# AlexandreRouma/SDRPlusPlus

Hardware: NVIDIA H100
Metric: complex IQ MSamples/s through FFT + 8-VFO WFM chain (higher is better)
Workload: dtype f32

## Files before the change

sdrplusplus_b200/csrc/api.cpp:

```cpp
#include "../../include/b200dsp.h"
#include "engine.h"
#include <chrono>
#include <map>
#include <cmath>
#include <cstdio>
#include <cstring>
#include <cstdlib>
#include <algorithm>

using namespace b200;

static int g_device = -1;

static int ensure_device() {
    int n = 0;
    cudaError_t e = cudaGetDeviceCount(&n);
    if (e != cudaSuccess || n <= 0) {
        set_error("no usable CUDA device (%s): libb200dsp has no CPU fallback", e == cudaSuccess ? "0 devices" : cudaGetErrorString(e));
        cudaGetLastError();
        return B200_ENODEV;
    }
    if (g_device < 0) { g_device = 0; }
    B200_CK(cudaSetDevice(g_device));
    return 0;
// ... 55 lines not shown
extern "C" int b200_resamp_plan_get(double inSR, double outSR, b200_resamp_plan* out) {
    if (!out) { set_error("null plan"); return B200_EINVAL; }
    ResampPlan pl = make_resamp_plan(inSR, outSR);
    memset(out, 0, sizeof(*out));
    out->mode = pl.mode;
    out->predec_ratio = pl.predec_ratio;
    out->interp = pl.interp;
    out->decim = pl.decim;
    out->ntaps = (int)pl.rtaps.size();
    out->taps_per_phase = pl.taps_per_phase;
    if (pl.use_decim) {
        const DecimPlan* dp = find_decim_plan(pl.predec_ratio);
        if (!dp) { set_error("no decimation plan for ratio %d", pl.predec_ratio); return B200_ENOPLAN; }
        out->nstages = (int)dp->stages.size();
        for (int i = 0; i < out->nstages && i < 8; i++) {
            out->stage_decim[i] = dp->stages[i].decim;
            out->stage_taps[i] = (int)dp->stages[i].taps.size();
        }
    }
    return 0;
}

static int bytes_per_sample(int fmt) { return fmt == B200_FMT_CF32 ? 8 : (fmt == B200_FMT_CS16 ? 4 : 2); }
static int ilog2(int n) { int l = 0; while ((1 << l) < n) { l++; } return l; }

struct FftCore {
    FftPlanDev plan;
    DevBuf tw, twf, win, work;
    int size = 0, nz = 0, window = 0;
    int create(int size_, int nz_, int window_, int max_batch = 1) {
        if (size_ < 8 || size_ > (1 << 22) || (size_ & (size_ - 1))) { set_error("FFT size %d must be a power of two in [8, 4194304]", size_); return B200_EINVAL; }
        if (nz_ < 1 || nz_ > size_) { set_error("bad nz %d", nz_); return B200_EINVAL; }
        size = size_; nz = nz_; window = window_;
        memset(&plan, 0, sizeof(plan));
        plan.N = size; plan.logN = ilog2(size);
        if (size <= 8192) { plan.N1 = size; plan.logN1 = plan.logN; plan.N2 = 1; plan.logN2 = 0; }
        else {
            plan.logN1 = (plan.logN + 1) / 2; plan.N1 = 1 << plan.logN1;
            plan.logN2 = plan.logN - plan.logN1; plan.N2 = 1 << plan.logN2;
        }
        plan.TW = std::max(plan.N1, plan.N2); plan.logTW = ilog2(plan.TW);
        std::vector<float2> t((size_t)plan.TW);
        for (int k = 0; k < plan.TW; k++) {
            double a = -2.0 * 3.14159265358979323846 * (double)k / (double)plan.TW;
            t[k] = make_float2((float)std::cos(a), (float)std::sin(a));
        }
        int rc;
        if ((rc = tw.alloc(t.size() * sizeof(float2)))) { return rc; }
        B200_CK(cudaMemcpy(tw.p, t.data(), t.size() * sizeof(float2), cudaMemcpyHostToDevice));
        std::vector<float> w = fft_window(window, nz);
        if ((rc = win.alloc((size_t)nz * sizeof(float)))) { return rc; }
        B200_CK(cudaMemcpy(win.p, w.data(), (size_t)nz * sizeof(float), cudaMemcpyHostToDevice));
        if ((rc = work.alloc((size_t)size * sizeof(float2) * (size_t)(max_batch > 0 ? max_batch : 1)))) { return rc; }
        plan.tw = tw.as<float2>(); plan.window = win.as<float>(); plan.nz = nz;
        plan.tw_fine = nullptr;
        if (plan.N2 > 1) {
            const int nf = size / plan.TW;
            std::vector<float2> f((size_t)nf);
            for (int j = 0; j < nf; j++) {
                double a = -2.0 * 3.14159265358979323846 * (double)j / (double)size;
                f[j] = make_float2((float)std::cos(a), (float)std::sin(a));
            }
            if ((rc = twf.alloc(f.size() * sizeof(float2)))) { return rc; }
            B200_CK(cudaMemcpy(twf.p, f.data(), f.size() * sizeof(float2), cudaMemcpyHostToDevice));
            plan.tw_fine = twf.as<float2>();
        }
        B200_CK(cudaDeviceSynchronize());
        return 0;
    }
};

struct VfoSlot {
    bool used = false;
    b200_vfo_cfg cfg;
    Chain chain;
    bool pend_offset = false, pend_bw = false;
    double new_offset = 0, new_bw = 0;
};

#define FE_SLOTS 4

struct b200_fe {
    double fs = 0;
    int max_chunk = 0;
    Scheduler sch;
    cudaStream_t own_stream = nullptr, copy_stream = nullptr, fft_stream = nullptr, tail_stream = nullptr, join_stream = nullptr;
    cudaEvent_t ev_tail_done[FE_SLOTS] = {};
    cudaEvent_t ev_fft_go = nullptr, ev_fft_done = nullptr, ev_lines_free = nullptr;
    bool overlap = true;
    bool lines_busy = false;
    float* lines_override = nullptr;
    bool fft_async = true;
    bool fft_join_pending = false;
    std::vector<std::unique_ptr<VfoSlot>> vfos;
    std::mutex mtx;
    DevBuf in_dev[FE_SLOTS];
    bool fft_on = false;
    FftCore fft;
    double fft_rate = 0;
    int skip = 0;
    DevBuf frame, lines;
    int max_lines = 0;
    unsigned long long pos = 0, fstart = 0;
    cudaEvent_t ev_h2d[FE_SLOTS] = {}, ev_compute[FE_SLOTS] = {}, ev_out[FE_SLOTS] = {};
    bool slot_used[FE_SLOTS] = {};
    int max_inflight = 2;
    unsigned long long nsub = 0, nwait = 0;
    int fft_serial = 0;
    int host_direct = -1;
    long long host_ns[4] = { 0, 0, 0, 0 };
    float scale16 = 1.0f / 32768.0f, scale8 = 1.0f / 128.0f;
    int decim = 1;
    double fs_eff = 0;
    bool dc_block = false, invert_iq = false;
    Chain pre;
    Scheduler sch_pre;
    DevBuf pp[FE_SLOTS];
    DevBuf dc_state, dc_segA, dc_segB;
    int max_eff = 0;
};

static float fe_ingest_scale(const b200_fe* fe, int fmt) {
    if (fmt == B200_FMT_CS16) { return fe->scale16; }
    if (fmt == B200_FMT_CS8) { return fe->scale8; }
    return 0.0f;
}

static int fe_alloc_fft(b200_fe* fe) {
    int rc;
    if ((rc = fe->frame.alloc((size_t)fe->fft.nz * sizeof(float2)))) { return rc; }
    long long interval = (long long)fe->fft.nz + fe->skip;
    fe->max_lines = (int)(fe->max_eff / interval) + 2;
    return fe->lines.alloc((size_t)fe->max_lines * fe->fft.size * sizeof(float));
}

extern "C" b200_fe* b200_fe_create(double samplerate, int max_chunk) {
    if (ensure_device()) { return nullptr; }
    if (samplerate <= 0 || max_chunk < 1) { set_error("bad samplerate/max_chunk"); return nullptr; }
    b200_fe* fe = new b200_fe;
    fe->fs = samplerate;
    fe->fs_eff = samplerate;
    fe->max_chunk = max_chunk;
    fe->max_eff = max_chunk;
    int lo = 0, hi = 0;
    cudaDeviceGetStreamPriorityRange(&lo, &hi);
    int pt = 2, pm = 1, pf = 0;
    if (const char* e = getenv("B200_STREAM_PRIO")) { sscanf(e, "%d,%d,%d", &pt, &pm, &pf); }
    if (const char* e = getenv("B200_FFT_SERIAL")) { fe->fft_serial = atoi(e); }
    if (const char* e = getenv("B200_FFT_CTA")) { kernels_set_fft_cta(atoi(e)); }
    auto prio = [&](int level) { int p = lo - level; return p < hi ? hi : p; };
    bool ok = cudaStreamCreateWithPriority(&fe->own_stream, cudaStreamNonBlocking, prio(pm)) == cudaSuccess &&
              cudaStreamCreateWithFlags(&fe->copy_stream, cudaStreamNonBlocking) == cudaSuccess &&
              cudaStreamCreateWithPriority(&fe->fft_stream, cudaStreamNonBlocking, prio(pf)) == cudaSuccess &&
              cudaStreamCreateWithPriority(&fe->tail_stream, cudaStreamNonBlocking, prio(pt)) == cudaSuccess &&
              cudaStreamCreateWithFlags(&fe->join_stream, cudaStreamNonBlocking) == cudaSuccess &&
              cudaEventCreateWithFlags(&fe->ev_lines_free, cudaEventDisableTiming) == cudaSuccess &&
              cudaEventCreateWithFlags(&fe->ev_fft_go, cudaEventDisableTiming) == cudaSuccess &&
              cudaEventCreateWithFlags(&fe->ev_fft_done, cudaEventDisableTiming) == cudaSuccess;
    for (int i = 0; i < FE_SLOTS && ok; i++) {
        ok = cudaEventCreateWithFlags(&fe->ev_h2d[i], cudaEventDisableTiming) == cudaSuccess &&
             cudaEventCreateWithFlags(&fe->ev_compute[i], cudaEventDisableTiming) == cudaSuccess &&
             cudaEventCreateWithFlags(&fe->ev_tail_done[i], cudaEventDisableTiming) == cudaSuccess &&
             cudaEventCreateWithFlags(&fe->ev_out[i], cudaEventDisableTiming) == cudaSuccess;
    }
    if (!ok || fe->sch.init_raw()) {
        if (ok) {} else { cuda_fail(cudaGetLastError(), "stream/event creation"); }
        b200_fe_destroy(fe);
        return nullptr;
    }
    fe->sch.stream = fe->own_stream;
    fe->sch.fuse.on = true;
    kernels_set_xd_tma_stages(2);
    kernels_set_xd_tma_diag(0);
    {
        int dev = 0, sms = 0;
        if (cudaGetDevice(&dev) == cudaSuccess && cudaDeviceGetAttribute(&sms, cudaDevAttrMultiProcessorCount, dev) == cudaSuccess && sms > 0) {
            fe->sch.sm_count = sms;
        }
    }
    if (fe->sch.enable_overlap(fe->tail_stream)) { b200_fe_destroy(fe); return nullptr; }
    return fe;
}

extern "C" void b200_fe_destroy(b200_fe* fe) {
    if (!fe) { return; }
    cudaDeviceSynchronize();
    for (int i = 0; i < FE_SLOTS; i++) {
        if (fe->ev_h2d[i]) { cudaEventDestroy(fe->ev_h2d[i]); }
        if (fe->ev_compute[i]) { cudaEventDestroy(fe->ev_compute[i]); }
        if (fe->ev_tail_done[i]) { cudaEventDestroy(fe->ev_tail_done[i]); }
        if (fe->ev_out[i]) { cudaEventDestroy(fe->ev_out[i]); }
    }
    if (fe->ev_lines_free) { cudaEventDestroy(fe->ev_lines_free); }
    if (fe->tail_stream) { cudaStreamDestroy(fe->tail_stream); }
    if (fe->join_stream) { cudaStreamDestroy(fe->join_stream); }
    for (int i = 0; i < 2; i++) {
        if (fe->sch.ev_stage1[i]) { cudaEventDestroy(fe->sch.ev_stage1[i]); }
        if (fe->sch.ev_tail[i]) { cudaEventDestroy(fe->sch.ev_tail[i]); }
    }
    if (fe->ev_fft_go) { cudaEventDestroy(fe->ev_fft_go); }
    if (fe->ev_fft_done) { cudaEventDestroy(fe->ev_fft_done); }
    if (fe->own_stream) { cudaStreamDestroy(fe->own_stream); }
// ... 162 lines not shown
    if (!v) { return B200_EINVAL; }
    return v->chain.max_out(count);
}
extern "C" int b200_fe_fft_max_lines(b200_fe* fe, int count) {
    if (!fe || !fe->fft_on) { return 0; }
    return (int)(count / ((long long)fe->fft.nz + fe->skip)) + 2;
}
extern "C" long long b200_fe_launch_count(b200_fe* fe) { return fe ? fe->sch.launches : 0; }
extern int g_xd_tma_launches;
extern "C" long long b200_fe_stat(b200_fe* fe, const char* key) {
    if (!fe || !key) { return -1; }
    if (!strcmp(key, "launches")) { return fe->sch.launches; }
    if (!strcmp(key, "s1_tma_launches")) { return g_xd_tma_launches; }
    if (!strcmp(key, "chunks")) { return (long long)fe->nsub; }
    if (!strcmp(key, "host_ns_plan")) { return fe->host_ns[0]; }
    if (!strcmp(key, "host_ns_fft")) { return fe->host_ns[1]; }
    if (!strcmp(key, "host_ns_run")) { return fe->host_ns[2]; }
    if (!strcmp(key, "host_ns_join")) { return fe->host_ns[3]; }
    if (!strcmp(key, "graph_hits")) { return fe->sch.graph_hits; }
    if (!strcmp(key, "graph_misses")) { return fe->sch.graph_misses; }
    if (!strcmp(key, "graphs")) { return (long long)fe->sch.graphs.size(); }
    if (!strcmp(key, "host_ns_stage1")) { return fe->sch.host_ns[0]; }
    if (!strcmp(key, "host_ns_tail")) { return fe->sch.host_ns[1]; }
    return -1;
}
extern "C" int b200_fe_set_option(b200_fe* fe, const char* key, int value) {
    if (!fe || !key) { set_error("null argument"); return B200_EINVAL; }
    if (!strcmp(key, "s1")) { fe->sch.s1_variant = value; return 0; }
    if (!strcmp(key, "overlap")) {
        if (b200_fe_vfo_count(fe) > 0) { set_error("'overlap' must be chosen before VFOs are added"); return B200_ESTATE; }
        if (cudaDeviceSynchronize() != cudaSuccess) { return cuda_fail(cudaGetLastError(), "sync"); }
        fe->sch.tail_stream = value ? fe->tail_stream : nullptr;
        return 0;
    }
    if (!strcmp(key, "pair")) { fe->sch.pair_conjugates = value != 0; return 0; }
    if (!strcmp(key, "fft_async")) { fe->fft_async = value != 0; return 0; }
    if (!strcmp(key, "s1_mt")) { kernels_set_xd_tile(value); return 0; }
    if (!strcmp(key, "s1_cps")) { kernels_set_xd_cps(value); return 0; }
    if (!strcmp(key, "s1_stages")) { kernels_set_xd_tma_stages(value); return 0; }
    if (!strcmp(key, "s1_diag")) { kernels_set_xd_tma_diag(value); return 0; }
    if (!strcmp(key, "s1_ctas")) { kernels_set_xd_tma_ctas(value); return 0; }
    if (!strcmp(key, "tails") || !strncmp(key, "ft_", 3)) {
        if (b200_fe_vfo_count(fe) > 0) { set_error("'%s' must be chosen before VFOs are added", key); return B200_ESTATE; }
        if (!strcmp(key, "tails")) { kernels_set_tail_variant(value >= 1 ? 1 : 0); fe->sch.fuse.on = value >= 2; return 0; }
        if (!strcmp(key, "ft_ob")) { fe->sch.fuse.ob_force = value; return 0; }
        if (!strcmp(key, "ft_obmax")) { fe->sch.fuse.ob_max = value; return 0; }
        if (!strcmp(key, "ft_smem_kb")) { fe->sch.fuse.smem_limit = value * 1024; return 0; }
        if (!strcmp(key, "ft_threads")) { fe->sch.fuse.threads = value; return 0; }
        if (!strcmp(key, "ft_direct")) { fe->sch.fuse.direct = value != 0; return 0; }
        if (!strcmp(key, "ft_prereg")) { fe->sch.fuse.pre_reg = value; return 0; }
        if (!strcmp(key, "ft_regall")) { fe->sch.fuse.reg_all = value != 0; return 0; }
    }
    if (!strcmp(key, "fft")) { kernels_set_fft_variant(value); return 0; }
    if (!strcmp(key, "fft_cta")) { kernels_set_fft_cta(value); return 0; }
    if (!strcmp(key, "host_direct")) { fe->host_direct = value; return 0; }
    if (!strcmp(key, "inflight")) {
        if (value < 1 || value > FE_SLOTS) { set_error("inflight: 1 ... %d", FE_SLOTS); return B200_EINVAL; }
        fe->max_inflight = value;
        return 0;
    }
    if (!strcmp(key, "fft_serial")) { fe->fft_serial = value; return 0; }
    if (!strcmp(key, "graph")) { fe->sch.graph_tails = value; if (value == 0) { fe->sch.drop_graphs(); } return 0; }
    if (!strcmp(key, "graph_max_count")) { fe->sch.graph_max_count = value; return 0; }
    if (!strcmp(key, "pdl")) { kernels_set_pdl(value); fe->sch.drop_graphs(); return 0; }
    if (!strcmp(key, "tail_split")) { fe->sch.tail_split = value; fe->sch.drop_graphs(); return 0; }
    if (!strcmp(key, "time_s1")) { fe->sch.time_s1 = value != 0; for (auto& t : fe->sch.timers) { t.used = 0; } return 0; }
    set_error("unknown option %s", key);
    return B200_EINVAL;
}

extern "C" int b200_fe_s1_stats(b200_fe* fe, double* ms_total, int* launches) {
    if (!fe || !ms_total || !launches) { set_error("null argument"); return B200_EINVAL; }
    return fe->sch.s1_stats(ms_total, launches);
}
extern "C" int b200_fe_group_stats(b200_fe* fe, int group, double* ms_total, int* launches) {
    if (!fe || !ms_total || !launches) { set_error("null argument"); return B200_EINVAL; }
    return fe->sch.group_stats(group, ms_total, launches);
}

extern "C" int b200_fe_reset(b200_fe* fe) {
    if (!fe) { set_error("null fe"); return B200_EINVAL; }
    std::lock_guard<std::mutex> lck(fe->mtx);
    B200_CK(cudaDeviceSynchronize());
    for (auto& v : fe->vfos) {
        if (v->used) { v->chain.reset_state(); }
    }
    int rc = fe->sch.reset_raw();
    if (!fe->pre.st.empty()) { fe->pre.reset_state(); }
    if (fe->dc_state.p) { B200_CK(cudaMemset(fe->dc_state.p, 0, 16)); B200_CK(cudaDeviceSynchronize()); }
    fe->pos = 0;
    fe->fstart = 0;
    return rc;
}

static std::mutex g_host_mtx;
static std::map<uintptr_t, size_t> g_host_allocs;
static bool host_buffer_is_ours(const void* p, size_t bytes) {
    std::lock_guard<std::mutex> lk(g_host_mtx);
    auto it = g_host_allocs.upper_bound((uintptr_t)p);
    if (it == g_host_allocs.begin()) { return false; }
    --it;
    return (uintptr_t)p + bytes <= it->first + it->second;
}

static inline long long host_clock_ns() {
    return (long long)std::chrono::duration_cast<std::chrono::nanoseconds>(std::chrono::steady_clock::now().time_since_epoch()).count();
}
// ... 1071 lines not shown
```

sdrplusplus_b200/csrc/fft_reg.cuh:

```cuda
#pragma once

__device__ constexpr float FR_COS[16] = { 1.000000000e+00f, 9.807852804e-01f, 9.238795325e-01f, 8.314696123e-01f, 7.071067812e-01f, 5.555702330e-01f,
                                          3.826834324e-01f, 1.950903220e-01f, 0.0f, -1.950903220e-01f, -3.826834324e-01f, -5.555702330e-01f,
                                          -7.071067812e-01f, -8.314696123e-01f, -9.238795325e-01f, -9.807852804e-01f };
__device__ constexpr float FR_SIN[16] = { 0.000000000e+00f, 1.950903220e-01f, 3.826834324e-01f, 5.555702330e-01f, 7.071067812e-01f, 8.314696123e-01f,
                                          9.238795325e-01f, 9.807852804e-01f, 1.0f, 9.807852804e-01f, 9.238795325e-01f, 8.314696123e-01f,
                                          7.071067812e-01f, 5.555702330e-01f, 3.826834324e-01f, 1.950903220e-01f };

template <int R, int K>
__device__ __forceinline__ float2 fr_mul_w(float2 v) {
    constexpr int k32 = K * (32 / R);
    if constexpr (k32 == 0) { return v; }
    else if constexpr (k32 == 8) { return make_float2(v.y, -v.x); }
    else if constexpr (k32 == 4) { return make_float2((v.x + v.y) * RSQRT2, (v.y - v.x) * RSQRT2); }
    else if constexpr (k32 == 12) { return make_float2((v.y - v.x) * RSQRT2, -(v.x + v.y) * RSQRT2); }
    else {
        constexpr float c = FR_COS[k32], s = FR_SIN[k32];
        return make_float2(fmaf(v.y, s, v.x * c), fmaf(-v.x, s, v.y * c));
    }
}
template <int R, int H, int I>
__device__ __forceinline__ void fr_stage(float2 (&a)[R]) {
    constexpr int blk = I / H, j = I % H, i0 = blk * 2 * H + j;
    const float2 u = a[i0], v = a[i0 + H];
    a[i0] = make_float2(u.x + v.x, u.y + v.y);
    a[i0 + H] = fr_mul_w<2 * H, j>(make_float2(u.x - v.x, u.y - v.y));
    if constexpr (I + 1 < R / 2) { fr_stage<R, H, I + 1>(a); }
    else if constexpr (H > 1) { fr_stage<R, H / 2, 0>(a); }
}
template <int R>
__device__ __forceinline__ void fr_dft(float2 (&a)[R]) { fr_stage<R, R / 2, 0>(a); }
template <int R>
__host__ __device__ constexpr int fr_brev(int c) {
    int r = 0;
    for (int bit = 1; bit < R; bit <<= 1) { r = (r << 1) | ((c & bit) ? 1 : 0); }
    return r;
}
template <int RA, int RB> struct FrGeom {
    static constexpr int n = RA * RB;
    static constexpr int TP = RA > RB ? RA : RB;
    static constexpr int crow = RB + 1;
    static constexpr int pitch = ((RA * crow + 13) / 16) * 16 + 2;
};

template <int RA, int RB>
__device__ __forceinline__ void fr_transform(float2 (&v)[RA > RB ? RA : RB], float2* ex, int t, const float2* __restrict__ tw, int twsh) {
    using G = FrGeom<RA, RB>;
    if (t < RB) {
        float2 a[RA];
#pragma unroll
        for (int i = 0; i < RA; i++) { a[i] = v[i]; }
        fr_dft<RA>(a);
#pragma unroll
        for (int c = 0; c < RA; c++) {
            float2 y = a[fr_brev<RA>(c)];
            if (c > 0) { y = cmulf(y, __ldg(tw + ((size_t)(t * c) << twsh))); }
            ex[c * G::crow + t] = y;
        }
    }
    __syncthreads();
    if (t < RA) {
        float2 b[RB];
#pragma unroll
        for (int i = 0; i < RB; i++) { b[i] = ex[t * G::crow + i]; }
        fr_dft<RB>(b);
#pragma unroll
        for (int i = 0; i < RB; i++) { v[i] = b[i]; }
    }
}

template <int FMT, int RA, int RB, int C, int MINB>
__global__ void __launch_bounds__(C * FrGeom<RA, RB>::TP, MINB) k_fftr_p1(const __grid_constant__ FftPlanDev pl, const void* __restrict__ src0,
                                                                    float2* __restrict__ work0, long long src_stride_bytes) {
    using G = FrGeom<RA, RB>;
    extern __shared__ __align__(16) float2 smem[];
    const int N2 = pl.N2;
    const void* src = reinterpret_cast<const char*>(src0) + (size_t)blockIdx.y * src_stride_bytes;
    float2* work = work0 + (size_t)blockIdx.y * pl.N;
    const int col = threadIdx.x % C, t = threadIdx.x / C;
    const int n2 = blockIdx.x * C + col;
    float2 v[G::TP];
    if (t < RB) {
#pragma unroll
        for (int a = 0; a < RA; a++) { v[a] = load_windowed<FMT>(pl, src, (a * RB + t) * N2 + n2); }
    }
    fr_transform<RA, RB>(v, smem + col * G::pitch, t, pl.tw, pl.logTW - pl.logN1);
    if (t < RA) {
        const int s = pl.logN - pl.logTW;
        const unsigned msk = (1u << s) - 1u;
#pragma unroll
        for (int d = 0; d < RB; d++) {
            const int k1 = t + RA * d;
            const unsigned e = (unsigned)k1 * (unsigned)n2;
            const float2 w = cmulf(__ldg(pl.tw + (e >> s)), __ldg(pl.tw_fine + (e & msk)));
            work[(size_t)k1 * N2 + n2] = cmulf(v[fr_brev<RB>(d)], w);
        }
    }
}

template <int RA, int RB, int R>
__global__ void __launch_bounds__(R * FrGeom<RA, RB>::TP) k_fftr_p2(const __grid_constant__ FftPlanDev pl, const float2* __restrict__ work0,
                                                                    float* __restrict__ out_db0) {
    using G = FrGeom<RA, RB>;
    extern __shared__ __align__(16) float2 smem[];
    const int N1 = pl.N1, N2 = pl.N2;
    const float2* work = work0 + (size_t)blockIdx.y * pl.N;
    float* out_db = out_db0 + (size_t)blockIdx.y * pl.N;
    const int t = threadIdx.x % G::TP, row = threadIdx.x / G::TP;
    const int r0 = blockIdx.x * R;
    float2 v[G::TP];
    if (t < RB) {
        const float2* __restrict__ p = work + (size_t)(r0 + row) * N2 + t;
#pragma unroll
        for (int a = 0; a < RA; a++) { v[a] = __ldg(p + a * RB); }
    }
    fr_transform<RA, RB>(v, smem + row * G::pitch, t, pl.tw, pl.logTW - pl.logN2);
    __syncthreads();
    float* T = reinterpret_cast<float*>(smem);
    const float nf = 1.0f / ((float)pl.N * (float)pl.N);
    if (t < RA) {
#pragma unroll
        for (int d = 0; d < RB; d++) { T[(t + RA * d) * (R + 1) + row] = power_db(v[fr_brev<RB>(d)], nf); }
    }
    __syncthreads();
    for (int idx = threadIdx.x; idx < G::n * R; idx += R * G::TP) {
        const int k2 = idx / R, rl = idx - k2 * R;
        out_db[(size_t)(r0 + rl) + (size_t)N1 * k2] = T[k2 * (R + 1) + rl];
    }
}
```

sdrplusplus_b200/csrc/kernels.cu:

```cuda
#include "kernels.cuh"
#include <unordered_map>
#include <mutex>
#include <math.h>
#include <string.h>
#include <algorithm>

template <int FMT>
__device__ __forceinline__ float2 load_iq(const void* __restrict__ p, long long i, float sc) {
    if (FMT == FMT_CF32) {
        return __ldg(reinterpret_cast<const float2*>(p) + i);
    }
    else if (FMT == FMT_CS16) {
        short2 v = __ldg(reinterpret_cast<const short2*>(p) + i);
        return make_float2((float)v.x * sc, (float)v.y * sc);
    }
    else {
        char2 v = __ldg(reinterpret_cast<const char2*>(p) + i);
        return make_float2((float)v.x * sc, (float)v.y * sc);
    }
}

template <int FMT>
__device__ __forceinline__ float2 load_x(const XdParams& p, long long i) {
    if (i >= 0) {
        if (i < p.count) { return load_iq<FMT>(p.in, i, p.in_scale); }
        return make_float2(0.0f, 0.0f);
    }
    long long h = (long long)p.hist_len + i;
    if (h >= 0) { return __ldg(p.hist + h); }
    return make_float2(0.0f, 0.0f);
}

__device__ __forceinline__ float2 phasor_u64(unsigned long long phase) {
    int hi = (int)(phase >> 32);
    float t = (float)hi * (1.0f / 2147483648.0f);
    float s, c;
    sincospif(t, &s, &c);
    return make_float2(c, s);
}

__device__ __forceinline__ float2 cmulf(float2 a, float2 b) {
    return make_float2(a.x * b.x - a.y * b.y, a.x * b.y + a.y * b.x);
}

__device__ __forceinline__ float2 ffma2(float2 a, float2 b, float2 c) {
    return make_float2(__fmaf_rn(a.x, b.x, c.x), __fmaf_rn(a.y, b.y, c.y));
}

__device__ __forceinline__ void pdl_trigger() { asm volatile("griddepcontrol.launch_dependents;" ::: "memory"); }
__device__ __forceinline__ void pdl_wait() { asm volatile("griddepcontrol.wait;" ::: "memory"); }
#define PDL_DEFAULT 2
static int g_pdl = -1;
int kernels_pdl() {
    if (g_pdl < 0) { const char* e = getenv("B200_PDL"); g_pdl = e ? atoi(e) : PDL_DEFAULT; if (g_pdl < 0 || g_pdl > 2) { g_pdl = PDL_DEFAULT; } }
    return g_pdl;
}
void kernels_set_pdl(int mode) { g_pdl = (mode >= 0 && mode <= 2) ? mode : PDL_DEFAULT; }
static int num_sms();
template <class P>
static cudaError_t launch_chain(void (*k)(const P), dim3 grid, dim3 block, size_t smem, cudaStream_t s, const P& p) {
    cudaLaunchConfig_t cfg;
    memset(&cfg, 0, sizeof(cfg));
    cfg.gridDim = grid; cfg.blockDim = block; cfg.dynamicSmemBytes = smem; cfg.stream = s;
    cudaLaunchAttribute at[1];
    const int mode = kernels_pdl();
    if (mode == 1 || (mode == 2 && (long long)grid.x * grid.y * grid.z <= 2LL * num_sms())) {
        at[0].id = cudaLaunchAttributeProgrammaticStreamSerialization;
        at[0].val.programmaticStreamSerializationAllowed = 1;
        cfg.attrs = at; cfg.numAttrs = 1;
    }
    return cudaLaunchKernelEx(&cfg, k, p);
}

template <int FMT>
__global__ void __launch_bounds__(128) k_xd_simple(const __grid_constant__ XdParams p) {
    const XdJob& J = p.job[blockIdx.y];
    int m = blockIdx.x * blockDim.x + threadIdx.x;
    if (m >= J.n_out) { return; }
    const int T = J.T;
    const long long i0 = (long long)J.offset + (long long)m * p.D - (T - 1);
    const float2* __restrict__ g = J.gpad + (p.D - 1);
    float ar = 0.0f, ai = 0.0f;
    for (int k = 0; k < T; k++) {
        float2 x = load_x<FMT>(p, i0 + k);
        float2 t = __ldg(g + k);
        ar += x.x * t.x - x.y * t.y;
        ai += x.x * t.y + x.y * t.x;
    }
    float2 ph = phasor_u64(J.phase0 + J.w * (unsigned long long)i0);
    J.out[m] = cmulf(make_float2(ar, ai), ph);
}

#define FL_M_PI_REF 3.1415926535f
#include "xd_pipe.cuh"
#include "xd_pfb.cuh"
#include "xd_tma.cuh"
#include "tails.cuh"
#include "dfir_reg.cuh"
#include "fused_tail.cuh"
#include "stereo.cuh"
#include "rds.cuh"

template <int FMT>
__global__ void __launch_bounds__(128) k_xd_edge(const __grid_constant__ XdParams p) {
    const XdJob& J = p.job[blockIdx.y];
    if (!J.retuned) { return; }
    int m = blockIdx.x * blockDim.x + threadIdx.x;
    if (m >= J.n_out) { return; }
    const int T = J.T;
    const long long i0 = (long long)J.offset + (long long)m * p.D - (T - 1);
    if (i0 >= 0) { return; }
    float ar = 0.0f, ai = 0.0f;
    for (int k = 0; k < T; k++) {
        long long i = i0 + k;
        float2 x = load_x<FMT>(p, i);
        unsigned long long ph = J.phase0 + ((i < 0) ? J.w_prev : J.w) * (unsigned long long)i;
        float2 z = cmulf(x, phasor_u64(ph));
        float t = __ldg(J.h + k);
        ar = fmaf(z.x, t, ar);
        ai = fmaf(z.y, t, ai);
    }
    J.out[m] = make_float2(ar, ai);
}

// ... 416 lines not shown
    const float2* work = work0 + (size_t)blockIdx.y * pl.N;
    float* out_db = out_db0 + (size_t)blockIdx.y * pl.N;
    const int pitch = N2 + 1;
    const int r0 = blockIdx.x * R;
#pragma unroll 4
    for (int t = threadIdx.x; t < R * N2; t += blockDim.x) {
        int rl = t / N2, n2 = t - rl * N2;
        smem[padf(rl * pitch + n2)] = __ldg(work + (size_t)(r0 + rl) * N2 + n2);
    }
    __syncthreads();
    fft_dif_smem<false>(smem, pl.logN2, R, pitch, pl.tw, pl.logTW);
    const float nf = 1.0f / ((float)pl.N * (float)pl.N);
    for (int t = threadIdx.x; t < R * N2; t += blockDim.x) {
        int k2 = t / R, rl = t - k2 * R;
        float2 X = smem[padf(rl * pitch + bitrev(k2, pl.logN2))];
        size_t k = (size_t)(r0 + rl) + (size_t)N1 * k2;
        out_db[k] = power_db(X, nf);
        if (out_raw) { out_raw[k] = X; }
    }
}

#include "fft_reg.cuh"
#include "preproc.cuh"

template <int FMT>
__global__ void __launch_bounds__(256) k_convert(const void* __restrict__ src, float2* __restrict__ dst, int n, float sc) {
    int i = blockIdx.x * blockDim.x + threadIdx.x;
    if (i < n) { dst[i] = load_iq<FMT>(src, i, sc); }
}

__global__ void __launch_bounds__(256) k_zoom_hold(const float* __restrict__ line, const int* __restrict__ start,
                                                     const int* __restrict__ len, int out_size, float* __restrict__ out,
                                                     float* hold, float hold_speed) {
    int i = blockIdx.x * blockDim.x + threadIdx.x;
    if (i >= out_size) { return; }
    float maxVal = -INFINITY;
    const int s = start[i], l = len[i];
    for (int j = 0; j < l; j++) {
        float v = __ldg(line + s + j);
        if (v > maxVal) { maxVal = v; }
    }
    out[i] = maxVal;
    if (hold && i >= 1) {
        float d = __fsub_rn(hold[i], hold_speed);
        hold[i] = (maxVal < d) ? d : maxVal;
    }
}

static int g_smem_optin = -1;
static int g_fft_variant = 1;
void kernels_set_fft_variant(int v) { g_fft_variant = v; }
int g_xd_tma_ctas = 0;
void kernels_set_xd_tma_ctas(int v) { g_xd_tma_ctas = v; }
static int g_fft_cta = 8;
void kernels_set_fft_cta(int v) { g_fft_cta = (v == 4) ? 4 : 8; }
int kernels_max_smem_optin() {
    if (g_smem_optin < 0) {
        int dev = 0, v = 0;
        cudaGetDevice(&dev);
        cudaDeviceGetAttribute(&v, cudaDevAttrMaxSharedMemoryPerBlockOptin, dev);
        g_smem_optin = v;
    }
    return g_smem_optin;
}

template <typename K>
static cudaError_t set_smem(K kernel, size_t bytes) {
    static std::mutex mtx;
    static std::unordered_map<const void*, size_t> have;
    std::lock_guard<std::mutex> lk(mtx);
    size_t& cur = have[(const void*)kernel];
    if (bytes <= cur) { return cudaSuccess; }
    cudaError_t e = cudaFuncSetAttribute(kernel, cudaFuncAttributeMaxDynamicSharedMemorySize, (int)bytes);
    if (e == cudaSuccess) { cur = bytes; }
    return e;
}

static inline int cdiv(long long a, long long b) { return (int)((a + b - 1) / b); }

#include "chanpfb.cuh"
#include "ifnr.cuh"
#include "tails_reg.cuh"


int g_xd_cps = 0;
void kernels_set_xd_cps(int v) { g_xd_cps = v; }
int g_xd_mt_override = 0;
void kernels_set_xd_tile(int mt) { g_xd_mt_override = mt; }
static int g_num_sms = -1;
static int num_sms() {
    if (g_num_sms < 0) {
        int dev = 0, v = 0;
        cudaGetDevice(&dev);
        cudaDeviceGetAttribute(&v, cudaDevAttrMultiProcessorCount, dev);
        g_num_sms = v > 0 ? v : 132;
    }
    return g_num_sms;
}

template <int FMT, int QC, int NT>
static cudaError_t launch_xd_pipe_t(const XdParams& p, const XpGeom& g, size_t smem, cudaStream_t s) {
    cudaError_t e = set_smem(k_xd_pipe<FMT, QC, NT>, smem);
    if (e != cudaSuccess) { return e; }
    int per_sm = (int)((size_t)233472 / (smem + 1024));
    if (per_sm > 2048 / NT) { per_sm = 2048 / NT; }
    if (per_sm > 512 / NT && NT >= 256) { per_sm = 512 / NT > 0 ? 512 / NT : 1; }
    if (NT == 128 && per_sm > 3) { per_sm = 3; }
    if (per_sm < 1) { per_sm = 1; }
// ... 403 lines not shown
    else if (threads == 256) { FT_LAUNCH(256, 1); }
    else { FT_LAUNCH(128, 0); }
#undef FT_LAUNCH
    return cudaGetLastError();
}
cudaError_t launch_fir_r(const FirRParams& p, cudaStream_t s) {
    if (p.max_out <= 0 || p.njobs <= 0) { return cudaSuccess; }
    if (g_tail_variant >= 1) {
        int maxT = 0;
        for (int v = 0; v < p.njobs; v++) { maxT = p.job[v].ntaps > maxT ? p.job[v].ntaps : maxT; }
        if (maxT <= TAIL_MAX_TAPS) {
            const int OB = FR2_THREADS * FR2_R;
            const int span = OB + maxT + FR2_R;
            size_t smem = ((size_t)maxT + (size_t)(span + (span >> 3) + 2)) * sizeof(float);
            cudaError_t e = set_smem(k_fir_r2, smem);
            if (e != cudaSuccess) { return e; }
            dim3 grid(cdiv(p.max_out, OB), p.njobs);
            k_fir_r2<<<grid, FR2_THREADS, smem, s>>>(p);
            return cudaGetLastError();
        }
    }
    dim3 grid(cdiv(p.max_out, 256), p.njobs);
    k_fir_r<<<grid, 256, 0, s>>>(p);
    return cudaGetLastError();
}
cudaError_t launch_seq(const SeqParams& p, cudaStream_t s) {
    if (p.njobs <= 0) { return cudaSuccess; }
    k_seq<<<p.njobs, 32, 0, s>>>(p);
    return cudaGetLastError();
}
cudaError_t launch_m2s(const M2SParams& p, cudaStream_t s) {
    if (p.max_n <= 0 || p.njobs <= 0) { return cudaSuccess; }
    dim3 grid(cdiv(p.max_n, 256), p.njobs);
    k_m2s<<<grid, 256, 0, s>>>(p);
    return cudaGetLastError();
}
cudaError_t launch_rxl(const RxlParams& p, cudaStream_t s) {
    if (p.max_n <= 0 || p.njobs <= 0) { return cudaSuccess; }
    dim3 grid(cdiv(p.max_n, 256), p.njobs);
    k_rxl<<<grid, 256, 0, s>>>(p);
    return cudaGetLastError();
}
cudaError_t launch_scale(const ScaleParams& p, cudaStream_t s) {
    if (p.max_n <= 0 || p.njobs <= 0) { return cudaSuccess; }
    dim3 grid(cdiv(p.max_n, 256), p.njobs);
    k_scale<<<grid, 256, 0, s>>>(p);
    return cudaGetLastError();
}
cudaError_t launch_carry(const CarryParams& p, cudaStream_t s) {
    if (p.njobs <= 0) { return cudaSuccess; }
    return launch_chain(k_carry, dim3((unsigned)p.njobs), dim3(256), 0, s, p);
}

template <int FMT>
static cudaError_t launch_fft_fmt(const FftPlanDev& pl, const void* src, float2* work, float* out_db, float2* out_raw,
                                  cudaStream_t s, int* nlaunch, int nbatch, long long src_stride_bytes) {
    cudaError_t e;
    if (pl.N1 == pl.N) {
        size_t smem = ((size_t)pl.N + (pl.N >> 4) + 2) * sizeof(float2);
        e = set_smem(k_fft_single<FMT>, smem);
        if (e != cudaSuccess) { return e; }
        int thr = pl.N / 8 < 32 ? 32 : (pl.N / 8 > 512 ? 512 : pl.N / 8);
        k_fft_single<FMT><<<dim3(1, nbatch), thr, smem, s>>>(pl, src, out_db, out_raw, src_stride_bytes);
        if (nlaunch) { (*nlaunch)++; }
        return cudaGetLastError();
    }
    if (g_fft_variant >= 1 && !out_raw && pl.tw_fine && pl.logN1 >= 8 && pl.logN1 <= 10 && pl.logN2 >= 8 && pl.logN2 <= 10) {
#define FR_P1(RA, RB, CC)                                                                                      \
        do {                                                                                                   \
            const size_t sm = (size_t)CC * FrGeom<RA, RB>::pitch * sizeof(float2);                             \
            e = set_smem(k_fftr_p1<FMT, RA, RB, CC, 2>, sm);                                                   \
            if (e != cudaSuccess) { return e; }                                                                \
            k_fftr_p1<FMT, RA, RB, CC, 2><<<dim3(pl.N2 / CC, nbatch), CC * FrGeom<RA, RB>::TP, sm, s>>>(pl, src, work, src_stride_bytes); \
        } while (0)
#define FR_P2(RA, RB, RR)                                                                                      \
        do {                                                                                                   \
            const size_t sm = (size_t)RR * FrGeom<RA, RB>::pitch * sizeof(float2);                             \
            e = set_smem(k_fftr_p2<RA, RB, RR>, sm);                                                           \
            if (e != cudaSuccess) { return e; }                                                                \
            k_fftr_p2<RA, RB, RR><<<dim3(pl.N1 / RR, nbatch), RR * FrGeom<RA, RB>::TP, sm, s>>>(pl, work, out_db); \
        } while (0)
        if (g_fft_cta == 4) {
            if (pl.logN1 == 10) { FR_P1(32, 32, 4); } else if (pl.logN1 == 9) { FR_P1(16, 32, 4); } else { FR_P1(16, 16, 4); }
        }
        else {
            if (pl.logN1 == 10) { FR_P1(32, 32, 8); } else if (pl.logN1 == 9) { FR_P1(16, 32, 8); } else { FR_P1(16, 16, 8); }
        }
        e = cudaGetLastError();
        if (e != cudaSuccess) { return e; }
        if (g_fft_cta == 4) {
            if (pl.logN2 == 10) { FR_P2(32, 32, 4); } else if (pl.logN2 == 9) { FR_P2(16, 32, 4); } else { FR_P2(16, 16, 4); }
        }
        else {
            if (pl.logN2 == 10) { FR_P2(32, 32, 8); } else if (pl.logN2 == 9) { FR_P2(16, 32, 8); } else { FR_P2(16, 16, 8); }
        }
#undef FR_P1
#undef FR_P2
        if (nlaunch) { (*nlaunch) += 2; }
        return cudaGetLastError();
    }
    int C = 16;
    while (C > 4 && (pl.N2 / C) * nbatch < 2 * num_sms()) { C >>= 1; }
    while ((size_t)pl.N1 * C * sizeof(float2) > 196608 && C > 1) { C >>= 1; }
    if (C > pl.N2) { C = pl.N2; }
    int R = 16;
    while (R > 4 && (pl.N1 / R) * nbatch < 2 * num_sms()) { R >>= 1; }
    while ((size_t)R * (pl.N2 + 1) * sizeof(float2) > 196608 && R > 1) { R >>= 1; }
    if (R > pl.N1) { R = pl.N1; }
    size_t smem1 = ((size_t)pl.N1 * C + ((size_t)pl.N1 * C >> 4) + 2) * sizeof(float2);
    size_t smem2 = ((size_t)R * (pl.N2 + 1) + ((size_t)R * (pl.N2 + 1) >> 4) + 2) * sizeof(float2);
    e = set_smem(k_fft_p1<FMT>, smem1);
    if (e != cudaSuccess) { return e; }
    e = set_smem(k_fft_p2, smem2);
    if (e != cudaSuccess) { return e; }
    const int thr1 = (pl.N1 / 8) * C >= 512 ? 512 : 256, thr2 = (pl.N2 / 8) * R >= 512 ? 512 : 256;
    k_fft_p1<FMT><<<dim3(pl.N2 / C, nbatch), thr1, smem1, s>>>(pl, src, work, C, src_stride_bytes);
    e = cudaGetLastError();
    if (e != cudaSuccess) { return e; }
    k_fft_p2<<<dim3(pl.N1 / R, nbatch), thr2, smem2, s>>>(pl, work, out_db, out_raw, R);
    if (nlaunch) { (*nlaunch) += 2; }
    return cudaGetLastError();
}

cudaError_t launch_fft_frames(const FftPlanDev& pl, const void* src, int fmt, float2* work, float* out_db,
                              float2* out_raw, cudaStream_t s, int* nlaunch, int nbatch, long long src_stride_bytes) {
    if (nbatch <= 0) { return cudaSuccess; }
    if (fmt == FMT_CF32) { return launch_fft_fmt<FMT_CF32>(pl, src, work, out_db, out_raw, s, nlaunch, nbatch, src_stride_bytes); }
    if (fmt == FMT_CS16) { return launch_fft_fmt<FMT_CS16>(pl, src, work, out_db, out_raw, s, nlaunch, nbatch, src_stride_bytes); }
    return launch_fft_fmt<FMT_CS8>(pl, src, work, out_db, out_raw, s, nlaunch, nbatch, src_stride_bytes);
}
cudaError_t launch_fft_frame(const FftPlanDev& pl, const void* src, int fmt, float2* work, float* out_db,
                             float2* out_raw, cudaStream_t s, int* nlaunch) {
    return launch_fft_frames(pl, src, fmt, work, out_db, out_raw, s, nlaunch, 1, 0);
}

cudaError_t launch_convert_cf32(const void* src, int fmt, float2* dst, int n, float scale, cudaStream_t s) {
    if (n <= 0) { return cudaSuccess; }
    int grid = cdiv(n, 256);
    if (fmt == FMT_CF32) { k_convert<FMT_CF32><<<grid, 256, 0, s>>>(src, dst, n, scale); }
    else if (fmt == FMT_CS16) { k_convert<FMT_CS16><<<grid, 256, 0, s>>>(src, dst, n, scale); }
    else { k_convert<FMT_CS8><<<grid, 256, 0, s>>>(src, dst, n, scale); }
    return cudaGetLastError();
}

__global__ void __launch_bounds__(256) k_export(const float* __restrict__ in, long long n, int type, float scalar, void* __restrict__ out) {
    const long long i = (long long)blockIdx.x * blockDim.x + threadIdx.x;
    if (i >= n) { return; }
    const float x = __ldg(in + i);
    if (type == EXP_U8) {
        const float v = __fadd_rn(__fmul_rn(x, 127.0f), 128.0f);
        reinterpret_cast<unsigned char*>(out)[i] = (unsigned char)__float2int_rz(v);
    }
// ... 60 lines not shown
```

sdrplusplus_b200/csrc/kernels.cuh:

```cuda
#pragma once
#include <cuda_runtime.h>
#include <stdint.h>

#define B200_BATCH 16

enum { FMT_CF32 = 0, FMT_CS16 = 1, FMT_CS8 = 2 };

struct XdJob {
    float2* out;
    const float2* gpad;
    unsigned long long phase0;
    unsigned long long w;
    int offset;
    int n_out;
    int T;
    const float* h;
    unsigned long long w_prev;
    int retuned;
};
struct XdParams {
    const void* in;
    const float2* hist;
    int hist_len;
    int count;
// ... 250 lines not shown

struct FftPlanDev {
    int N, logN;
    int N1, logN1;
    int N2, logN2;
    const float2* tw;
    int TW, logTW;
    const float2* tw_fine;
    const float* window;
    float in_scale;
    int nz;
};

cudaError_t launch_xlate_decim(const XdParams& p, int fmt, int variant, cudaStream_t s, int* nlaunch);
cudaError_t launch_xd_edge(const XdParams& p, int fmt, cudaStream_t s, int* nlaunch);
cudaError_t launch_fir_c(const FirParams& p, cudaStream_t s);
cudaError_t launch_fir_reg(const FirParams& p, cudaStream_t s);
cudaError_t launch_firr_reg(const FirRParams& p, cudaStream_t s);
cudaError_t launch_poly(const PolyParams& p, cudaStream_t s);
cudaError_t launch_quad(const QuadParams& p, cudaStream_t s);
cudaError_t launch_fir_r(const FirRParams& p, cudaStream_t s);
cudaError_t launch_seq(const SeqParams& p, cudaStream_t s);
cudaError_t launch_m2s(const M2SParams& p, cudaStream_t s);
cudaError_t launch_scale(const ScaleParams& p, cudaStream_t s);
cudaError_t launch_carry(const CarryParams& p, cudaStream_t s);
cudaError_t launch_fft_frame(const FftPlanDev& pl, const void* src, int fmt, float2* work, float* out_db,
                             float2* out_raw, cudaStream_t s, int* nlaunch);
cudaError_t launch_fft_frames(const FftPlanDev& pl, const void* src, int fmt, float2* work, float* out_db,
                              float2* out_raw, cudaStream_t s, int* nlaunch, int nbatch, long long src_stride_bytes);
struct DcbParams {
    const void* in;
    float2* out;
    int fmt;
    int count;
    float in_scale;
    float rate;
    int dc_on, conj_on;
    float2* state;
    float2* segB;
    float* segA;
    int nseg;
};
cudaError_t launch_preproc(const DcbParams& p, cudaStream_t s, int* nlaunch);
cudaError_t launch_convert_cf32(const void* src, int fmt, float2* dst, int n, float scale, cudaStream_t s);
enum { EXP_U8 = 0, EXP_I8 = 1, EXP_I16 = 2, EXP_I32 = 3 };
cudaError_t launch_export(const float* in, long long n, int type, float scalar, void* out, cudaStream_t s);
cudaError_t launch_index_max(const float* in, long long n, float* out_val, cudaStream_t s);
cudaError_t launch_zoom_hold_tbl(const float* line, const int* start, const int* len, int out_size, float* out,
                                 float* hold, float hold_speed, cudaStream_t s);
int kernels_max_smem_optin();
void kernels_set_tail_variant(int v);
void kernels_set_fft_variant(int v);
void kernels_set_xd_tma_ctas(int v);
void kernels_set_fft_cta(int v);
void kernels_set_xd_tile(int mt);
void kernels_set_xd_tma_diag(int v);
void kernels_set_xd_tma_stages(int n);
void kernels_set_xd_cps(int v);
```

Baseline: 84440.

## Run register FFT per frame with L2-resident scratch, cache hints and PDL chaining

Replaces the batched two-pass register FFT launch with a per-frame loop that reuses a single frame-sized work buffer. Pass 1 stores with an L2 evict_last policy, and pass 2 loads with evict_first and then discards the scratch lines so they are never written back to DRAM. Launches are chained with programmatic dependent launch so each pass can overlap the previous one's tail. The intent is to keep the intermediate transpose in L2 instead of DRAM, at the cost of twice as many launches per batch and serialised frames. The fft_cta=4 option is removed.

After: 87980 (median of 6 runs). 1.04x the previous value.

```diff
diff --git a/sdrplusplus_b200/csrc/api.cpp b/sdrplusplus_b200/csrc/api.cpp
--- a/sdrplusplus_b200/csrc/api.cpp
+++ b/sdrplusplus_b200/csrc/api.cpp
@@ -131,6 +131,7 @@
         if ((rc = win.alloc((size_t)nz * sizeof(float)))) { return rc; }
         B200_CK(cudaMemcpy(win.p, w.data(), (size_t)nz * sizeof(float), cudaMemcpyHostToDevice));
         if ((rc = work.alloc((size_t)size * sizeof(float2) * (size_t)(max_batch > 0 ? max_batch : 1)))) { return rc; }
+        if ((uintptr_t)work.p & 127) { set_error("FFT work buffer not 128-byte aligned"); return B200_ECUDA; }
         plan.tw = tw.as<float2>(); plan.window = win.as<float>(); plan.nz = nz;
         plan.tw_fine = nullptr;
         if (plan.N2 > 1) {
@@ -226,7 +227,6 @@
     int pt = 2, pm = 1, pf = 0;
     if (const char* e = getenv("B200_STREAM_PRIO")) { sscanf(e, "%d,%d,%d", &pt, &pm, &pf); }
     if (const char* e = getenv("B200_FFT_SERIAL")) { fe->fft_serial = atoi(e); }
-    if (const char* e = getenv("B200_FFT_CTA")) { kernels_set_fft_cta(atoi(e)); }
     auto prio = [&](int level) { int p = lo - level; return p < hi ? hi : p; };
     bool ok = cudaStreamCreateWithPriority(&fe->own_stream, cudaStreamNonBlocking, prio(pm)) == cudaSuccess &&
               cudaStreamCreateWithFlags(&fe->copy_stream, cudaStreamNonBlocking) == cudaSuccess &&
@@ -495,7 +495,6 @@
         if (!strcmp(key, "ft_regall")) { fe->sch.fuse.reg_all = value != 0; return 0; }
     }
     if (!strcmp(key, "fft")) { kernels_set_fft_variant(value); return 0; }
-    if (!strcmp(key, "fft_cta")) { kernels_set_fft_cta(value); return 0; }
     if (!strcmp(key, "host_direct")) { fe->host_direct = value; return 0; }
     if (!strcmp(key, "inflight")) {
         if (value < 1 || value > FE_SLOTS) { set_error("inflight: 1 ... %d", FE_SLOTS); return B200_EINVAL; }
diff --git a/sdrplusplus_b200/csrc/fft_reg.cuh b/sdrplusplus_b200/csrc/fft_reg.cuh
--- a/sdrplusplus_b200/csrc/fft_reg.cuh
+++ b/sdrplusplus_b200/csrc/fft_reg.cuh
@@ -69,14 +69,32 @@
     }
 }
 
-template <int FMT, int RA, int RB, int C, int MINB>
-__global__ void __launch_bounds__(C * FrGeom<RA, RB>::TP, MINB) k_fftr_p1(const __grid_constant__ FftPlanDev pl, const void* __restrict__ src0,
-                                                                    float2* __restrict__ work0, long long src_stride_bytes) {
+__device__ __forceinline__ unsigned long long l2_policy_evict_last() {
+    unsigned long long pol;
+    asm volatile("createpolicy.fractional.L2::evict_last.b64 %0, 1.0;" : "=l"(pol));
+    return pol;
+}
+__device__ __forceinline__ unsigned long long l2_policy_evict_first() {
+    unsigned long long pol;
+    asm volatile("createpolicy.fractional.L2::evict_first.b64 %0, 1.0;" : "=l"(pol));
+    return pol;
+}
+__device__ __forceinline__ void st_l2_hint(float2* p, float2 v, unsigned long long pol) {
+    asm volatile("st.global.L2::cache_hint.v2.f32 [%0], {%1, %2}, %3;" ::"l"(p), "f"(v.x), "f"(v.y), "l"(pol) : "memory");
+}
+__device__ __forceinline__ float2 ld_cg_l2_hint(const float2* p, unsigned long long pol) {
+    float2 v;
+    asm volatile("ld.global.cg.L2::cache_hint.v2.f32 {%0, %1}, [%2], %3;" : "=f"(v.x), "=f"(v.y) : "l"(p), "l"(pol) : "memory");
+    return v;
+}
+__device__ __forceinline__ void l2_discard_line(const void* p) { asm volatile("discard.global.L2 [%0], 128;" ::"l"(p) : "memory"); }
+
+template <int FMT, int RA, int RB, int C>
+__global__ void __launch_bounds__(C * FrGeom<RA, RB>::TP, 2) k_fftr_p1(const __grid_constant__ FftPlanDev pl, const void* __restrict__ src,
+                                                                       float2* __restrict__ work) {
     using G = FrGeom<RA, RB>;
     extern __shared__ __align__(16) float2 smem[];
     const int N2 = pl.N2;
-    const void* src = reinterpret_cast<const char*>(src0) + (size_t)blockIdx.y * src_stride_bytes;
-    float2* work = work0 + (size_t)blockIdx.y * pl.N;
     const int col = threadIdx.x % C, t = threadIdx.x / C;
     const int n2 = blockIdx.x * C + col;
     float2 v[G::TP];
@@ -85,7 +103,9 @@
         for (int a = 0; a < RA; a++) { v[a] = load_windowed<FMT>(pl, src, (a * RB + t) * N2 + n2); }
     }
     fr_transform<RA, RB>(v, smem + col * G::pitch, t, pl.tw, pl.logTW - pl.logN1);
+    pdl_wait();
     if (t < RA) {
+        const unsigned long long pol = l2_policy_evict_last();
         const int s = pl.logN - pl.logTW;
         const unsigned msk = (1u << s) - 1u;
 #pragma unroll
@@ -93,29 +113,33 @@
             const int k1 = t + RA * d;
             const unsigned e = (unsigned)k1 * (unsigned)n2;
             const float2 w = cmulf(__ldg(pl.tw + (e >> s)), __ldg(pl.tw_fine + (e & msk)));
-            work[(size_t)k1 * N2 + n2] = cmulf(v[fr_brev<RB>(d)], w);
+            st_l2_hint(work + (size_t)k1 * N2 + n2, cmulf(v[fr_brev<RB>(d)], w), pol);
         }
     }
+    pdl_trigger();
 }
 
 template <int RA, int RB, int R>
-__global__ void __launch_bounds__(R * FrGeom<RA, RB>::TP) k_fftr_p2(const __grid_constant__ FftPlanDev pl, const float2* __restrict__ work0,
-                                                                    float* __restrict__ out_db0) {
+__global__ void __launch_bounds__(R * FrGeom<RA, RB>::TP) k_fftr_p2(const __grid_constant__ FftPlanDev pl, float2* __restrict__ work,
+                                                                    float* __restrict__ out_db) {
     using G = FrGeom<RA, RB>;
     extern __shared__ __align__(16) float2 smem[];
     const int N1 = pl.N1, N2 = pl.N2;
-    const float2* work = work0 + (size_t)blockIdx.y * pl.N;
-    float* out_db = out_db0 + (size_t)blockIdx.y * pl.N;
     const int t = threadIdx.x % G::TP, row = threadIdx.x / G::TP;
     const int r0 = blockIdx.x * R;
+    pdl_wait();
+    pdl_trigger();
     float2 v[G::TP];
     if (t < RB) {
-        const float2* __restrict__ p = work + (size_t)(r0 + row) * N2 + t;
+        const unsigned long long pol = l2_policy_evict_first();
+        const float2* p = work + (size_t)(r0 + row) * N2 + t;
 #pragma unroll
-        for (int a = 0; a < RA; a++) { v[a] = __ldg(p + a * RB); }
+        for (int a = 0; a < RA; a++) { v[a] = ld_cg_l2_hint(p + a * RB, pol); }
     }
     fr_transform<RA, RB>(v, smem + row * G::pitch, t, pl.tw, pl.logTW - pl.logN2);
     __syncthreads();
+    const char* rows = reinterpret_cast<const char*>(work + (size_t)r0 * N2);
+    for (int l = threadIdx.x; l < R * N2 * (int)sizeof(float2) / 128; l += R * G::TP) { l2_discard_line(rows + (size_t)l * 128); }
     float* T = reinterpret_cast<float*>(smem);
     const float nf = 1.0f / ((float)pl.N * (float)pl.N);
     if (t < RA) {
diff --git a/sdrplusplus_b200/csrc/kernels.cu b/sdrplusplus_b200/csrc/kernels.cu
--- a/sdrplusplus_b200/csrc/kernels.cu
+++ b/sdrplusplus_b200/csrc/kernels.cu
@@ -57,8 +57,8 @@
 }
 void kernels_set_pdl(int mode) { g_pdl = (mode >= 0 && mode <= 2) ? mode : PDL_DEFAULT; }
 static int num_sms();
-template <class P>
-static cudaError_t launch_chain(void (*k)(const P), dim3 grid, dim3 block, size_t smem, cudaStream_t s, const P& p) {
+template <class... KArgs, class... Args>
+static cudaError_t launch_chain(void (*k)(KArgs...), dim3 grid, dim3 block, size_t smem, cudaStream_t s, const Args&... args) {
     cudaLaunchConfig_t cfg;
     memset(&cfg, 0, sizeof(cfg));
     cfg.gridDim = grid; cfg.blockDim = block; cfg.dynamicSmemBytes = smem; cfg.stream = s;
@@ -69,7 +69,7 @@
         at[0].val.programmaticStreamSerializationAllowed = 1;
         cfg.attrs = at; cfg.numAttrs = 1;
     }
-    return cudaLaunchKernelEx(&cfg, k, p);
+    return cudaLaunchKernelEx(&cfg, k, args...);
 }
 
 template <int FMT>
@@ -592,8 +592,6 @@
 void kernels_set_fft_variant(int v) { g_fft_variant = v; }
 int g_xd_tma_ctas = 0;
 void kernels_set_xd_tma_ctas(int v) { g_xd_tma_ctas = v; }
-static int g_fft_cta = 8;
-void kernels_set_fft_cta(int v) { g_fft_cta = (v == 4) ? 4 : 8; }
 int kernels_max_smem_optin() {
     if (g_smem_optin < 0) {
         int dev = 0, v = 0;
@@ -1103,6 +1101,43 @@
     return launch_chain(k_carry, dim3((unsigned)p.njobs), dim3(256), 0, s, p);
 }
 
+#define FR_CTA 8
+template <int FMT, int RA, int RB>
+static cudaError_t launch_fftr_p1(const FftPlanDev& pl, const void* src, float2* work, cudaStream_t s, bool pdl) {
+    const size_t sm = (size_t)FR_CTA * FrGeom<RA, RB>::pitch * sizeof(float2);
+    cudaError_t e = set_smem(k_fftr_p1<FMT, RA, RB, FR_CTA>, sm);
+    if (e != cudaSuccess) { return e; }
+    const dim3 grid(pl.N2 / FR_CTA), block(FR_CTA * FrGeom<RA, RB>::TP);
+    if (pdl) { return launch_chain(k_fftr_p1<FMT, RA, RB, FR_CTA>, grid, block, sm, s, pl, src, work); }
+    k_fftr_p1<FMT, RA, RB, FR_CTA><<<grid, block, sm, s>>>(pl, src, work);
+    return cudaGetLastError();
+}
+template <int RA, int RB>
+static cudaError_t launch_fftr_p2(const FftPlanDev& pl, float2* work, float* out_db, cudaStream_t s) {
+    const size_t sm = (size_t)FR_CTA * FrGeom<RA, RB>::pitch * sizeof(float2);
+    cudaError_t e = set_smem(k_fftr_p2<RA, RB, FR_CTA>, sm);
+    if (e != cudaSuccess) { return e; }
+    return launch_chain(k_fftr_p2<RA, RB, FR_CTA>, dim3(pl.N1 / FR_CTA), dim3(FR_CTA * FrGeom<RA, RB>::TP), sm, s, pl, work, out_db);
+}
+template <int FMT>
+static cudaError_t launch_fftr_frames(const FftPlanDev& pl, const void* src, float2* work, float* out_db, cudaStream_t s,
+                                      int* nlaunch, int nbatch, long long src_stride_bytes) {
+    cudaError_t e = cudaSuccess;
+    for (int f = 0; f < nbatch && e == cudaSuccess; f++) {
+        const void* fsrc = reinterpret_cast<const char*>(src) + (size_t)f * src_stride_bytes;
+        if (pl.logN1 == 10) { e = launch_fftr_p1<FMT, 32, 32>(pl, fsrc, work, s, f > 0); }
+        else if (pl.logN1 == 9) { e = launch_fftr_p1<FMT, 16, 32>(pl, fsrc, work, s, f > 0); }
+        else { e = launch_fftr_p1<FMT, 16, 16>(pl, fsrc, work, s, f > 0); }
+        if (e != cudaSuccess) { break; }
+        float* db = out_db + (size_t)f * pl.N;
+        if (pl.logN2 == 10) { e = launch_fftr_p2<32, 32>(pl, work, db, s); }
+        else if (pl.logN2 == 9) { e = launch_fftr_p2<16, 32>(pl, work, db, s); }
+        else { e = launch_fftr_p2<16, 16>(pl, work, db, s); }
+        if (nlaunch) { (*nlaunch) += 2; }
+    }
+    return e;
+}
+
 template <int FMT>
 static cudaError_t launch_fft_fmt(const FftPlanDev& pl, const void* src, float2* work, float* out_db, float2* out_raw,
                                   cudaStream_t s, int* nlaunch, int nbatch, long long src_stride_bytes) {
@@ -1117,38 +1152,7 @@
         return cudaGetLastError();
     }
     if (g_fft_variant >= 1 && !out_raw && pl.tw_fine && pl.logN1 >= 8 && pl.logN1 <= 10 && pl.logN2 >= 8 && pl.logN2 <= 10) {
-#define FR_P1(RA, RB, CC)                                                                                      \
-        do {                                                                                                   \
-            const size_t sm = (size_t)CC * FrGeom<RA, RB>::pitch * sizeof(float2);                             \
-            e = set_smem(k_fftr_p1<FMT, RA, RB, CC, 2>, sm);                                                   \
-            if (e != cudaSuccess) { return e; }                                                                \
-            k_fftr_p1<FMT, RA, RB, CC, 2><<<dim3(pl.N2 / CC, nbatch), CC * FrGeom<RA, RB>::TP, sm, s>>>(pl, src, work, src_stride_bytes); \
-        } while (0)
-#define FR_P2(RA, RB, RR)                                                                                      \
-        do {                                                                                                   \
-            const size_t sm = (size_t)RR * FrGeom<RA, RB>::pitch * sizeof(float2);                             \
-            e = set_smem(k_fftr_p2<RA, RB, RR>, sm);                                                           \
-            if (e != cudaSuccess) { return e; }                                                                \
-            k_fftr_p2<RA, RB, RR><<<dim3(pl.N1 / RR, nbatch), RR * FrGeom<RA, RB>::TP, sm, s>>>(pl, work, out_db); \
-        } while (0)
-        if (g_fft_cta == 4) {
-            if (pl.logN1 == 10) { FR_P1(32, 32, 4); } else if (pl.logN1 == 9) { FR_P1(16, 32, 4); } else { FR_P1(16, 16, 4); }
-        }
-        else {
-            if (pl.logN1 == 10) { FR_P1(32, 32, 8); } else if (pl.logN1 == 9) { FR_P1(16, 32, 8); } else { FR_P1(16, 16, 8); }
-        }
-        e = cudaGetLastError();
-        if (e != cudaSuccess) { return e; }
-        if (g_fft_cta == 4) {
-            if (pl.logN2 == 10) { FR_P2(32, 32, 4); } else if (pl.logN2 == 9) { FR_P2(16, 32, 4); } else { FR_P2(16, 16, 4); }
-        }
-        else {
-            if (pl.logN2 == 10) { FR_P2(32, 32, 8); } else if (pl.logN2 == 9) { FR_P2(16, 32, 8); } else { FR_P2(16, 16, 8); }
-        }
-#undef FR_P1
-#undef FR_P2
-        if (nlaunch) { (*nlaunch) += 2; }
-        return cudaGetLastError();
+        return launch_fftr_frames<FMT>(pl, src, work, out_db, s, nlaunch, nbatch, src_stride_bytes);
     }
     int C = 16;
     while (C > 4 && (pl.N2 / C) * nbatch < 2 * num_sms()) { C >>= 1; }
diff --git a/sdrplusplus_b200/csrc/kernels.cuh b/sdrplusplus_b200/csrc/kernels.cuh
--- a/sdrplusplus_b200/csrc/kernels.cuh
+++ b/sdrplusplus_b200/csrc/kernels.cuh
@@ -326,7 +326,6 @@
 void kernels_set_tail_variant(int v);
 void kernels_set_fft_variant(int v);
 void kernels_set_xd_tma_ctas(int v);
-void kernels_set_fft_cta(int v);
 void kernels_set_xd_tile(int mt);
 void kernels_set_xd_tma_diag(int v);
 void kernels_set_xd_tma_stages(int n);
```
